# A511-1103/building-detection

Hardware: AMD Instinct MI355X
Metric: 512x512 tiles/sec fwd+bwd DeepLabv3+ (v3plus.py) (full train step: fwd+loss+bwd+Adam) (higher is better)
Workload: dtype f32; 1 GPU; DeepLabv3+ (v3plus.py) 512x512 bs=16/GPU fp32, train step, single GPU; global_batch=16, train_step=one hipGraph replay per step (compile(jit_compile=True)), side_stream_filter_gradients=True

## Files before the change

### building_detection_amd/_lib.py

```python
from __future__ import annotations

import ctypes as C
import os
import threading

_HERE = os.path.dirname(os.path.abspath(__file__))
LIB_PATH = os.path.join(_HERE, "libsegengine.so")

SG_F32, SG_BF16, SG_I64 = 0, 1, 2
SG_HEAD_F32 = 0x100
SG_COMM_ID_BYTES = 128
SG_EPI_BIAS, SG_EPI_RELU = 1, 2
SG_PRO_UP2, SG_EPI_DOWN2 = 16, 32
SG_X_UP2 = 0x200
SG_ACT_RELU, SG_ACT_SIGMOID = 0, 1
SG_LOSS_CE2, SG_LOSS_FOCAL, SG_LOSS_EDGE_FOCAL = 0, 1, 2
SG_MAX_CLASSES = 32
SG_AUGMENT_MAX_ITEMS = 64
SG_AUG_FLIP_UD, SG_AUG_FLIP_LR, SG_AUG_SWAP_RB, SG_AUG_THRESHOLD = 1, 2, 4, 8
SG_SCENE_MAX_ITEMS = 64
SG_SYM_FLIP_UD, SG_SYM_FLIP_LR, SG_SYM_TRANSPOSE = 1, 2, 4
SG_OPT_ADAM, SG_OPT_SGD = 0, 1
SG_OPT_AMSGRAD, SG_OPT_NESTEROV, SG_OPT_EMA = 1, 2, 4
SG_OPT_CLIP_NONE, SG_OPT_CLIP_VALUE, SG_OPT_CLIP_NORM, SG_OPT_CLIP_GLOBAL = 0, 1, 2, 3
# ... 227 lines not shown

_SIGNATURES = {
    "sg_abi_version": (_i, []),
    "sg_last_error": (C.c_char_p, []),
    "sg_set_conv_x6": (_i, [_i]),
    "sg_create": (_i, [_i, _pp]),
    "sg_destroy": (_i, [_vp]),
    "sg_num_cus": (_i, [_vp]),
    "sg_conv2d_fwd": (_i, [_vp, _vp, _i, _dp, _vp, _vp, _vp, _vp, _i, _op]),
    "sg_conv2d_fwd_ws_bytes": (_sz, [_dp]),
    "sg_conv2d_fwd_stats_bytes": (_sz, [_dp]),
    "sg_get_conv_x6": (_i, []),
    "sg_conv2d_planes_job": (_i, [_vp, _i, _dp, _i, C.POINTER(PlanesJob), C.POINTER(C.c_size_t)]),
    "sg_prepare_planes": (_i, [_vp, _vp, _vp, _vp, _vp, _i, _i]),
    "sg_bn_tiles_ws_bytes": (_sz, [_vp, _i, _i]),
    "sg_bn_train_fwd_tiles": (_i, [_vp, _vp, _i, _i64, _i, _vp, _i, _vp, _vp, _vp, _vp, C.c_float, C.c_float, _i, _vp, _sz]),
    "sg_bn_apply": (_i, [_vp, _vp, _i, _i64, _i, _vp, _vp, _vp, _vp, _vp, _vp, _i]),
    "sg_conv2d_dgrad_ws_bytes": (_sz, [_dp]),
    "sg_conv2d_dgrad": (_i, [_vp, _vp, _i, _dp, _vp, _vp, _vp, _vp, _i, _op]),
    "sg_conv2d_wgrad_ws_bytes": (_sz, [_vp, _dp]),
    "sg_conv2d_wgrad": (_i, [_vp, _vp, _i, _dp, _vp, _vp, _vp, _vp, _op]),
    "sg_conv2d_caps": (_i, [_vp, _i, _dp, _i, C.POINTER(ConvCaps)]),
    "sg_conv2d_plan": (_i, [_vp, _i, _dp, _i, _i, _i, C.POINTER(ConvPlan)]),
    "sg_split_planes": (_i, [_vp, _vp, _vp, _i64, _i, _i, _vp]),
    "sg_conv2d_wgrad_planes_ws_bytes": (_sz, [_vp, _dp]),
    "sg_conv2d_wgrad_planes": (_i, [_vp, _vp, _dp, _vp, _vp, _vp, _vp, _sz]),
    "sg_conv2d_wgrad_plan": (_i, [_vp, _i, _dp, _i, _i, C.POINTER(WgradPlan)]),
    "sg_bias_grad_ws_bytes": (_sz, [_vp, _i64, _i]),
    "sg_bias_grad": (_i, [_vp, _vp, _i, _i64, _i, _i, _vp, _vp, _vp, _sz]),
    "sg_dwconv2d_fwd": (_i, [_vp, _vp, _i, _dp, _vp, _vp, _vp, _i, C.POINTER(BnIn)]),
    "sg_dwconv2d_dgrad": (_i, [_vp, _vp, _i, _dp, _vp, _vp, _vp, _vp, _i, _vp, C.POINTER(DwBnSums)]),
    "sg_dwconv2d_dgrad_bnsums_ws_bytes": (_sz, [_vp, _dp]),
    "sg_dwconv2d_wgrad_ws_bytes": (_sz, [_vp, _dp]),
    "sg_dwconv2d_wgrad": (_i, [_vp, _vp, _i, _dp, _vp, _vp, _vp, _i, C.POINTER(BnIn), _vp, _sz]),
    "sg_dwconv2d_plan": (_i, [_vp, _i, _dp, _i, _i, _i, C.POINTER(DwPlan)]),
    "sg_dense_fwd": (_i, [_vp, _vp, _i, _i, _i, _i, _vp, _vp, _vp, _vp, _i]),
    "sg_bn_ws_bytes": (_sz, [_vp, _i64, _i]),
    "sg_bn_train_fwd": (_i, [_vp, _vp, _i, _i64, _i, _vp, _vp, _vp, _vp, _vp, _vp, _vp, _vp, _f, _f, _i, _i, _vp, _sz]),
    "sg_bn_train_bwd": (_i, [_vp, _vp, _i, _i64, _i, _vp, _vp, _vp, _vp, _vp, _vp, _vp, _vp, _vp, _vp, _i, _vp, _sz]),
    "sg_bn_train_bwd_apply": (_i, [_vp, _vp, _i, _i64, _i] + [_vp] * 9 + [_i]),
    "sg_bn_train_bwd_thin_ok": (_i, [_vp, _i, _i64, _i, _i, _i]),
    "sg_bn_train_bwd_thin": (_i, [_vp, _vp, _i, _i64, _i, _i, _i] + [_vp] * 10 + [_i, _vp, _sz]),
    "sg_bn_infer": (_i, [_vp, _vp, _i, _i64, _i, _vp, _vp, _vp, _vp, _vp, _vp, _f, _i]),
    "sg_add2_bn": (_i, [_vp, _vp, _i, _i64, _i] + [_vp] * 11 + [_i, _i, _f, _i, _i]),
    "sg_bn_plan": (_i, [_vp, _i, _i64, _i, _i, _i, C.POINTER(BnPlan)]),
    "sg_seg_plan": (_i, [_vp, _i, _i, _i64, _i, _i, _i, C.POINTER(SegPlan)]),
# ... 146 lines not shown
```

### building_detection_amd/csrc/conv_common.h

```cpp
#pragma once
#include "sg_common.h"
#include <stdlib.h>
#include <string.h>
#include <type_traits>

namespace sgconv {

constexpr int BM = 128;
constexpr int BK = 32;
constexpr int LDA = BK + 4;

template <int V>
using IC = std::integral_constant<int, V>;

struct BnIn {
  const float* mean;
  const float* invstd;
  const float* gamma;
  const float* beta;
  int relu, infer;
  float eps;
};
__device__ __forceinline__ f32x4 bn_in_inv(const BnIn& b, int c) {
  f32x4 is = *reinterpret_cast<const f32x4*>(b.invstd + c);
// ... 27 lines not shown
  const float* __restrict__ bias;
  float* __restrict__ y;
  int H, W, C, x_ld;
  int OH, OW;
  int Nout, y_ld;
  int a_mul, k_mul, off_h, off_w, div;
  int K, M;
  int flags;
  int stagger;
  int ablate;
  uint32_t x_bytes, w_bytes;
  int skip_taps;
  int group_m;
  int cb;
  FastDiv fd_ohow, fd_ow, fd_c, fd_kw;
  const unsigned short* __restrict__ wq;
  int Kpad, Npad;
  int kd;
  float* __restrict__ stats;
  int perm2;
  FastDiv fd_mc, fd_hcwc, fd_wc;
  const float* res;
  const unsigned short* a_planes;
  BnIn bn;
  BnBwdIn bnb;
};

__device__ __forceinline__ int spt_of(const IgemmParams& p) { return p.C / BK; }

__device__ __forceinline__ void row_to_pixel(const IgemmParams& p, uint32_t m, uint32_t& n, uint32_t& oh, uint32_t& ow) {
  if (p.perm2) {
    uint32_t cls, r, rem, i, j;
    fd_divmod(m, p.fd_mc, cls, r);
    fd_divmod(r, p.fd_hcwc, n, rem);
    fd_divmod(rem, p.fd_wc, i, j);
    oh = 2 * i + (cls >> 1);
    ow = 2 * j + (cls & 1);
  } else {
    uint32_t rem;
    fd_divmod(m, p.fd_ohow, n, rem);
    fd_divmod(rem, p.fd_ow, oh, ow);
  }
}
__device__ __forceinline__ int64_t row_to_yoff(const IgemmParams& p, int row) {
  if (!p.perm2) return (int64_t)row * p.y_ld;
  uint32_t n, oh, ow;
  row_to_pixel(p, (uint32_t)row, n, oh, ow);
  return ((int64_t)(n * p.OH + oh) * p.OW + ow) * p.y_ld;
}

struct WgradParams {
  const float* __restrict__ x;
  const float* __restrict__ dy;
  float* __restrict__ out;
  int H, W, Cin, x_ld;
  int OH, OW, Cout, y_ld;
  int stride, dil, pad_t, pad_l;
  int K, P;
  int slabs_per_split;
  int stagger;
  uint32_t x_bytes, dy_bytes;
  int skip_slabs;
  int KH_KW;
  int tap_inner;
  uint32_t x_plane_bytes, dy_plane_bytes;
  BnIn bn;
  int up;
  FastDiv fd_ohow, fd_ow, fd_c, fd_kw, fd_oh;
};

typedef __bf16 bf16x8_t __attribute__((ext_vector_type(8)));
// ... 95 lines not shown
  plan_common(p, vec, bn);
  return bn;
}

enum ConvFamily {
  CONV_NATIVE,
  CONV_THIN,
  CONV_HEAD,
  CONV_SLAB,
  CONV_PATCH,
  CONV_WIDE
};
constexpr int PLAN_NOT_THIN = 1 << 30;

struct ConvPlan {
  ConvFamily family = CONV_NATIVE;
  int nb = 0;
  bool vec = false;
  int perm2 = 0;
  int npl = 0, Ck = 0, Ckp = 0, K = 0, kd = 0, Kpad = 0, Npad = 0, nblocks = 0;
  int wbn = 0;
  size_t w_bytes = 0;
  int x6w_S = 0, b16w_S = 0;
  bool deep = false;
  size_t a_img_bytes = 0, part_img_bytes = 0;
  bool res = false;
  bool bn_in = false;
  bool up2 = false;
  bool bnb = false;
  bool planes_in = false;

  size_t scratch_bytes(int images) const {
    return (((size_t)images * a_img_bytes + 255) & ~(size_t)255) + (size_t)images * part_img_bytes;
  }
  size_t ws_bytes(int images) const {
    const size_t sc = scratch_bytes(images);
    return sc ? ((w_bytes + 255) & ~(size_t)255) + sc : w_bytes;
  }
};

inline SlabKernel slab_kernel_of(const ConvPlan& pl, bool b16, bool with_res) {
  if (pl.npl == 3 && !b16 && pl.x6w_S > 0 && !with_res) return SLAB_X6W;
  if (b16 && pl.deep) return (pl.b16w_S > 0 && !with_res) ? SLAB_B16W : SLAB_B16;
  return SLAB_X6;
}
inline void slab_fill(IgemmParams& p, const ConvPlan& pl) {
// ... 58 lines not shown
```

### building_detection_amd/csrc/conv_igemm.hip

```cpp
#include "conv_common.h"
#include "conv_native.h"
#include "conv_thin.h"
#include "conv_x6p.h"
#include "conv_x6wp.h"

using namespace sgconv;

namespace {

int g_x6_mode = -1;

#include "conv_x6.h"
#include "conv_b16.h"
#include "conv_pw.h"
#include "conv_b16w.h"
#include "conv_x6w.h"

inline int x6_var_of(int64_t tiles, int num_cus) {
  const int var = x6_variant();
  return var < 0 ? ((tiles <= 3 * (int64_t)num_cus) ? 1 : 0) : var;
}
inline bool x6_mf16_of(const IgemmParams& p) { return sg_switch<SW_X6_MF16>() && p.K != p.C; }

template <int NPL, typename TA>
// ... 47 lines not shown
        if constexpr (NPL == 3) {
          if (p.bnb.x)
            return pl.wbn == 256 ? launch_pw_wide<NPL, TA, 256, true>(p, st) : launch_pw_wide<NPL, TA, 384, true>(p, st);
        }
        return pl.wbn == 256 ? launch_pw_wide<NPL, TA, 256>(p, st) : launch_pw_wide<NPL, TA, 384>(p, st);
      }
      break;
    case CONV_SLAB: {
      const int Ck = p.C;
      slab_fill(p, pl);
      p.wq = (const unsigned short*)ws;
      if (!prepared) {
        dim3 grid((unsigned)(p.Kpad / 32), (unsigned)(p.Npad / 32));
        hipLaunchKernelGGL(split3_weights_kernel, grid, dim3(256), 0, st, w, (unsigned short*)ws, pl.K, N, p.Kpad, p.Npad, Ck,
                           Cin * Cout, dgrad ? 1 : Cout, dgrad ? Cout : 1, NPL, pl.Ckp, p.kd);
        SG_LAUNCH_CHECK("split3_weights_kernel");
      }
      char* scratch = (char*)ws + ((pl.w_bytes + 255) & ~(size_t)255);
      const SlabKernel sk = slab_kernel_of(pl, B16, p.res != nullptr);
      if constexpr (NPL == 3 && !B16) {
        if (sk == SLAB_X6W) {
          IgemmParams q = p;
          slab_common(q, sk, 4, num_cus);
          q.ablate = sg_switch<SW_X6W_ABLATE>();
          return launch_x6w(q, pl.x6w_S, scratch, st);
        }
      }
      if constexpr (NPL == 1 && B16) {
        if (sk == SLAB_B16W) {
          IgemmParams q = p;
          slab_common(q, sk, 2, num_cus);
          return launch_b16w(q, pl.b16w_S, pl.b16w_S > 1 ? reinterpret_cast<float*>(scratch) : nullptr, st);
        }
        if (sk == SLAB_B16) return dispatch_b16(p, num_cus, st);
      }
      if (sk != SLAB_X6) break;
      return dispatch_x6<NPL, TA>(p, num_cus, st);
    }
    default:
      break;
  }
  sg_set_error("run_x6: kernel family %d does not read weight planes in this arithmetic (%d planes)", (int)pl.family, NPL);
  return SG_EINVAL;
}

inline size_t x6_ws_bytes(int taps, int C, int N) {
// ... 22 lines not shown
                     int flags, int eb) {
  p.x = (const float*)x;
  p.w = (const float*)w;
  p.bias = (const float*)bias;
  p.y = (float*)y;
  p.H = d->H; p.W = d->W; p.C = d->Cin; p.x_ld = d->x_ld ? d->x_ld : d->Cin;
  p.OH = d->Ho; p.OW = d->Wo;
  p.Nout = d->Cout; p.y_ld = d->y_ld ? d->y_ld : d->Cout;
  p.a_mul = d->stride; p.k_mul = d->dilation; p.off_h = -d->pad_t; p.off_w = -d->pad_l; p.div = 1;
  p.K = d->KH * d->KW * d->Cin;
  p.M = d->N * d->Ho * d->Wo;
  p.flags = flags;
  p.fd_ohow = make_fastdiv((uint32_t)(d->Ho * d->Wo));
  p.fd_ow = make_fastdiv((uint32_t)d->Wo);
  p.fd_c = make_fastdiv((uint32_t)d->Cin);
  p.fd_kw = make_fastdiv((uint32_t)d->KW);
  const int64_t xb = (((int64_t)d->N * d->H * d->W - 1) * p.x_ld + d->Cin) * eb, wb = (int64_t)p.K * d->Cout * 4;
  p.x_bytes = xb < (1ll << 31) ? (uint32_t)xb : 0;
  p.w_bytes = wb < (1ll << 31) ? (uint32_t)wb : 0;
  p.stats = nullptr;
  p.perm2 = 0;
  p.res = nullptr;
  p.a_planes = nullptr;
  p.bn.mean = nullptr;
  p.bnb.x = nullptr;
}

void fill_dgrad_params(IgemmParams& p, const sg_conv_desc* d, const void* dy, const void* wt, const void* bias, void* dx,
                       int flags, int eb) {
  p.x = (const float*)dy;
  p.w = (const float*)wt;
  p.bias = (const float*)bias;
  p.y = (float*)dx;
  p.H = d->Ho; p.W = d->Wo; p.C = d->Cout; p.x_ld = d->y_ld ? d->y_ld : d->Cout;
  p.OH = d->H; p.OW = d->W;
  p.Nout = d->Cin; p.y_ld = d->x_ld ? d->x_ld : d->Cin;
  p.a_mul = 1; p.k_mul = -d->dilation; p.off_h = d->pad_t; p.off_w = d->pad_l; p.div = d->stride;
  p.K = d->KH * d->KW * d->Cout;
  p.M = d->N * d->H * d->W;
  p.flags = flags;
  p.fd_ohow = make_fastdiv((uint32_t)(d->H * d->W));
  p.fd_ow = make_fastdiv((uint32_t)d->W);
  p.fd_c = make_fastdiv((uint32_t)d->Cout);
  p.fd_kw = make_fastdiv((uint32_t)d->KW);
  const int64_t xb = (((int64_t)d->N * d->Ho * d->Wo - 1) * p.x_ld + d->Cout) * eb, wb = (int64_t)p.K * d->Cin * 4;
  p.x_bytes = xb < (1ll << 31) ? (uint32_t)xb : 0;
  p.w_bytes = wb < (1ll << 31) ? (uint32_t)wb : 0;
  p.stats = nullptr;
  p.perm2 = 0;
  p.res = nullptr;
  p.a_planes = nullptr;
  p.bn.mean = nullptr;
  p.bnb.x = nullptr;
}

ConvPlan plan_conv_mode(int mode, int dtype, const sg_conv_desc* d, bool dgrad, int flags) {
  ConvPlan pl;
  const bool b16 = dt_storage(dtype) == SG_BF16, head32 = (dtype & SG_HEAD_F32) != 0;
  const bool f32 = dt_storage(dtype) == SG_F32 && !head32;
  const int eb = dt_bytes(dtype);
  const bool x_dense = !d->x_ld || d->x_ld == d->Cin, y_dense = !d->y_ld || d->y_ld == d->Cout;
  pl.up2 = f32 && mode == 1 && x6p_up2_geom(d) && x6wp_geom(d);
  const bool thin = thin_ok(d) && !(flags & PLAN_NOT_THIN) && !(dgrad && (flags & (SG_EPI_BIAS | SG_EPI_RELU)));
  if (head32) {
    pl.family = thin ? CONV_THIN : CONV_HEAD;
    pl.nb = thin ? d->N : images_per_2gib(d, 2, 4);
    return pl;
  }
  pl.nb = images_per_2gib(d, eb, eb);
  if (thin) {
    pl.family = CONV_THIN;
    pl.res = dgrad;
    pl.bn_in = !dgrad && f32 && !(dtype & SG_X_UP2) && x_dense;
    return pl;
// ... 47 lines not shown
  pl.family = CONV_SLAB;
  pl.res = dgrad;
  pl.deep = b16 && sg_switch<SW_B16_DEEP>();
  pl.kd = x6_plane_kd(b16, pl.Ckp, pl.K == pl.Ckp);
  pl.Kpad = x6_kpad(pl.K, pl.kd);
  pl.Npad = x6_npad(N);
  pl.nblocks = (pl.Kpad / 32) * (pl.Npad / 32);
  pl.w_bytes = x6_planes_bytes(pl.K, N, pl.npl, pl.kd);
  const size_t img_part = (size_t)g.OH * g.OW * N * sizeof(float);
  if (pl.npl == 3 && pl.kd == XW_KD && xw > 0) {
    pl.x6w_S = xw;
    pl.a_img_bytes = (size_t)3 * g.H * g.W * g.C * 2;
    pl.part_img_bytes = xw > 1 ? xw * img_part : 0;
    pl.planes_in = pl.Ckp == pl.Ck && x_dense && y_dense;
  }
  if (pl.deep && pl.kd == BW_KD) {
    pl.b16w_S = b16w_shares(g);
    pl.part_img_bytes = pl.b16w_S > 1 ? pl.b16w_S * img_part : 0;
  }
  return pl;
}

ConvPlan plan_conv(int num_cus, int dtype, const sg_conv_desc* d, bool dgrad, int flags) {
  (void)num_cus;
  return plan_conv_mode(x6_mode(), dtype, d, dgrad, flags);
}

inline void wgrad_extents(int dtype, const sg_conv_desc* d, uint32_t& x_bytes, uint32_t& dy_bytes) {
  const int up = (dtype & SG_X_UP2) ? 1 : 0, eb = dt_bytes(dtype), eby = (dtype & SG_HEAD_F32) ? 4 : eb;
  const int64_t xl = d->x_ld ? d->x_ld : d->Cin, yl = d->y_ld ? d->y_ld : d->Cout;
  const int64_t xb = (((int64_t)d->N * (d->H >> up) * (d->W >> up) - 1) * xl + d->Cin) * eb;
  const int64_t yb = (((int64_t)d->N * d->Ho * d->Wo - 1) * yl + d->Cout) * eby;
  x_bytes = xb < (1ll << 31) ? (uint32_t)xb : 0;
  dy_bytes = yb < (1ll << 31) ? (uint32_t)yb : 0;
}

static int wgrad_slab_split(int num_cus, const sg_conv_desc* d, bool b16) {
  const int64_t K = (int64_t)d->KH * d->KW * d->Cin, P = (int64_t)d->N * d->Ho * d->Wo;
  const int bn = wgrad_bn(d->Cout);
  const int64_t tiles = sg_cdiv(K, BM) * sg_cdiv(d->Cout, bn);
  const int64_t nslab = sg_cdiv(P, BK);
  const int64_t slots = 2 * (int64_t)num_cus;
  const double flops = 2.0 * (double)tiles * BM * bn * (double)P;
  const bool x6_rate = (wgrad_x6_geom(d) || (d->stride == 2 && d->dilation == 1 && d->Wo % BK == 0 && d->Cout >= 16)) && d->Cin % 4 == 0;
  const double rate_x6 = sg_switch_f<SW_WGRAD_PLAN_RATE>() * 1e12;
  const double rate_b16 = sg_switch_f<SW_WGRAD_PLAN_RATE_B16>() * 1e12;
  const double rate = x6_rate ? (b16 ? rate_b16 : rate_x6) : 110e12;
  int64_t maxS = nslab / 8;
// ... 615 lines not shown
  ConvPlan pl = plan_conv(ctx->num_cus, dtype, d, dg, flags);
  if (pl.family == CONV_THIN && !thin_operands_ok(pl, d, aligned == 16, ebx)) pl = plan_conv(ctx->num_cus, dtype, d, dg, flags | PLAN_NOT_THIN);
  if (pl.family == CONV_HEAD) SG_CHECK_ARG(pl.nb >= 1, "%s: one image of the softmax head beyond 2 GiB", who);
  const int nb = (pl.nb >= 1 && pl.nb < d->N) ? pl.nb : d->N;
  const bool fast = pl.family >= CONV_SLAB && pl.vec && aligned == 16;
  sg_conv_plan o;
  memset(&o, 0, sizeof(o));
  o.family = (int)pl.family;
  o.fast = fast;
  o.nb = nb;
  o.nsub = (int)sg_cdiv(d->N, nb);
  o.tail_n = d->N - (o.nsub - 1) * nb;
  o.vec = pl.vec; o.perm2 = pl.perm2; o.npl = pl.npl; o.kd = pl.kd; o.Ck = pl.Ck; o.Ckp = pl.Ckp; o.wbn = pl.wbn;
  o.x6w_S = pl.x6w_S; o.b16w_S = pl.b16w_S; o.deep = pl.deep;
  o.res = pl.res; o.bn_in = pl.bn_in; o.up2 = pl.up2; o.bnb = pl.bnb; o.planes_in = pl.planes_in;
  o.ws_bytes = pl.ws_bytes(nb);
  sg_conv_desc sub = *d;
  sub.N = nb;
  o.main = conv_launch_form(ctx->num_cus, dtype, &sub, pl, fast, dg, aligned, false);
  if (dg && pl.res && !head32 && (pl.family == CONV_THIN || fast)) o.with_res = conv_launch_form(ctx->num_cus, dtype, &sub, pl, fast, dg, aligned, true);
  sub.N = o.tail_n;
  o.tail = conv_launch_form(ctx->num_cus, dtype, &sub, pl, fast, dg, aligned, false);
  *out = o;
  return 0;
}

static int wgrad_plan_checked(const sg_ctx* ctx, int dtype, const sg_conv_desc* d, int ax, int ay, bool planes, const char* who, WgradPlan* pl) {
  SG_CHECK_ARG(ctx != nullptr, "%s: null ctx", who);
  SG_CHECK_ARG(dt_ok(dtype), "%s: dtype %d", who, dtype);
  int rc = check_desc(d, who);
  if (rc) return rc;
  const bool b16 = dt_storage(dtype) == SG_BF16, head32 = (dtype & SG_HEAD_F32) != 0;
  SG_CHECK_ARG(!head32 || (b16 && d->Cout <= 4), "%s: SG_HEAD_F32 needs Cout <= 4 (a softmax head) on bf16 storage", who);
  SG_CHECK_ARG(!planes || (dtype == SG_F32 && ax == 16 && ay == 16), "%s: null / unaligned tensor", who);
  *pl = plan_wgrad(ctx->num_cus, dtype, d, ax, ay, planes);
  if (planes && !pl->main.family) {
    sg_set_error("%s: geometry outside the planes-in kernel (stride 1 SAME, W %% 32 = 0, channels %% 8 = 0, dense "
                 "planes below 2 GiB, not a wide pointwise / patch-form layer, x6 arithmetic)", who);
    return SG_EUNSUPPORTED;
  }
  SG_CHECK_ARG(!(head32 && pl->chunks > 1), "%s: softmax head beyond 2 GiB", who);
  return 0;
}

int sg_conv2d_wgrad_plan(const sg_ctx* ctx, int dtype, const sg_conv_desc* d, int aligned, int planes, sg_wgrad_plan* out) {
  SG_CHECK_ARG(out != nullptr, "sg_conv2d_wgrad_plan: null out");
// ... 214 lines not shown
```

### building_detection_amd/csrc/conv_x6w.h

```cpp
#pragma once

constexpr int XW_M = 128, XW_N = 256, XW_KD = 32, XW_RB = 64;
constexpr int XW_A = 3 * XW_M * XW_RB;
constexpr int XW_B = 3 * XW_N * XW_RB;
constexpr int XW_STAGE = XW_A + XW_B;
constexpr int XW_LDS = 2 * XW_STAGE;

__device__ __forceinline__ int xw_swz(int row) { return (row >> 2) & 3; }

__global__ __launch_bounds__(256) void x6w_split_kernel(const float* __restrict__ x, unsigned short* __restrict__ planes, int64_t rows,
                                                        int C, int x_ld) {
  const int cq = C / 4;
  const int64_t total = rows * cq, plane = rows * (int64_t)C;
  const int64_t stride = (int64_t)gridDim.x * blockDim.x;
  for (int64_t i = (int64_t)blockIdx.x * blockDim.x + threadIdx.x; i < total; i += stride) {
    const int64_t r = i / cq;
    const int c = (int)(i - r * cq) * 4;
    const f32x4 f = *reinterpret_cast<const f32x4*>(x + r * x_ld + c);
    unsigned h0, m0, l0, h1, m1, l1;
    split3_pair(f[0], f[1], h0, m0, l0);
    split3_pair(f[2], f[3], h1, m1, l1);
    unsigned short* dst = planes + r * C + c;
    *reinterpret_cast<u32x2_t*>(dst) = (u32x2_t){h0, h1};
    *reinterpret_cast<u32x2_t*>(dst + plane) = (u32x2_t){m0, m1};
// ... 18 lines not shown
  if (p.group_m > 1) {
    const uint32_t ntm = ntiles / ntn, gm = (uint32_t)p.group_m;
    const uint32_t per = gm * ntn, g = bid / per, r = bid - g * per;
    const uint32_t left = ntm - g * gm, gsz = left < gm ? left : gm;
    tile_n = r / gsz;
    tile_m = g * gm + (r - tile_n * gsz);
  } else {
    tile_m = bid / ntn;
    tile_n = bid - tile_m * ntn;
  }
  const int m0 = tile_m * XW_M, n0 = tile_n * XW_N;

  const __amdgpu_buffer_rsrc_t rsrc_a = __builtin_amdgcn_make_buffer_rsrc(const_cast<unsigned short*>(aq), 0, (int)aq_bytes, 0x00020000);
  const __amdgpu_buffer_rsrc_t rsrc_w =
      __builtin_amdgcn_make_buffer_rsrc(const_cast<unsigned short*>(p.wq), 0, (int)p.w_bytes, 0x00020000);

  const int a_row = wave * 16 + (lane >> 2);
  const int a_chunk = 16 * ((lane & 3) ^ xw_swz(a_row));
  int a_lin = 0, a_hw = (int)0x80008000u;
  {
    const int m = m0 + a_row;
    if (m < p.M) {
      uint32_t n, oh, ow;
      row_to_pixel(p, (uint32_t)m, n, oh, ow);
      const int ohs = (int)oh * p.a_mul + p.off_h, ows = (int)ow * p.a_mul + p.off_w;
      a_lin = (int)n * p.H * p.W + ohs * p.W + ows;
      a_hw = (ohs << 16) | (ows & 0xffff);
    }
  }
  unsigned b_voff[6];
  const int kblocks = p.Kpad >> 5;
#pragma unroll
  for (int j = 0; j < 6; ++j) {
    const int idx = wave + 8 * j;
    const int pl = idx >> 4, rb = idx & 15;
    const int row = rb * 16 + (lane >> 2);
    const int c = (lane & 3) ^ xw_swz(row);
    const int nrow = n0 + row;
    b_voff[j] = nrow < p.Npad ? (unsigned)((((int64_t)pl * kblocks) * p.Npad + nrow) * XW_RB + 16 * c) : OOB;
  }
  auto tap_valid = [&](int dh, int dw, int& pix) -> bool {
    const int ohs = a_hw >> 16, ows = (int)(short)(a_hw & 0xffff);
    const int ih = ohs + dh, iw = ows + dw;
    pix = a_lin + dh * p.W + dw;
    return ((unsigned)ih < (unsigned)p.H) && ((unsigned)iw < (unsigned)p.W);
  };

// ... 174 lines not shown
          __builtin_amdgcn_sched_group_barrier(0x100, 1, 0);
        }
#pragma unroll
        for (int g = 0; g < 9; ++g) {
          __builtin_amdgcn_sched_group_barrier(0x008, 1, 0);
          __builtin_amdgcn_sched_group_barrier(0x020, 1, 0);
        }
        __builtin_amdgcn_sched_group_barrier(0x008, 3, 0);
        __builtin_amdgcn_sched_barrier(0);
      }
      asm volatile("s_waitcnt vmcnt(0)" ::: "memory");
    }
  }

  const bool whole = S == 1;
  const bool has_bias = whole && (p.flags & SG_EPI_BIAS) != 0;
  const bool do_relu = whole && (p.flags & SG_EPI_RELU) != 0;
  {
    float* dst = whole ? p.y : part + (int64_t)split * ((int64_t)p.M * p.Nout);
    const int ld = whole ? p.y_ld : p.Nout;
    const uint32_t obytes = (uint32_t)((((int64_t)p.M - 1) * ld + p.Nout) * 4);
    const __amdgpu_buffer_rsrc_t rsrc_o = __builtin_amdgcn_make_buffer_rsrc(dst, 0, (int)obytes, 0x00020000);
    const unsigned row0 = (unsigned)(m0 + wm + 4 * lh);
#pragma unroll
    for (int j = 0; j < TN; ++j) {
      const int col = n0 + wn + 32 * j + lr;
      const bool cv = col < p.Nout;
      const float bv = has_bias ? p.bias[cv ? col : p.Nout - 1] : 0.f;
      const unsigned cterm = cv ? (unsigned)col * 4u : OOB;
#pragma unroll
      for (int i = 0; i < TM; ++i)
#pragma unroll
        for (int r = 0; r < 16; ++r) {
          const unsigned row = row0 + 32 * i + (r & 3) + 8 * (r >> 2);
          float v = acc[i][j][r] + bv;
          v = do_relu ? fmaxf(v, 0.f) : v;
          unsigned voff = cterm + row * (unsigned)ld * 4u;
          voff = row < (unsigned)p.M ? voff : OOB;
          __builtin_amdgcn_raw_buffer_store_b32(__builtin_bit_cast(unsigned, v), rsrc_o, (int)voff, 0, 0);
        }
    }
  }

  if (whole && p.stats) {
    float* red = reinterpret_cast<float*>(smem);
    float* tmean = red + 2 * XW_N;
    const int nvalid = (p.M - m0) < XW_M ? (p.M - m0) : XW_M;
    const bool hb = (p.flags & SG_EPI_BIAS) != 0;
    __syncthreads();
#pragma unroll
    for (int pass = 0; pass < 2; ++pass) {
#pragma unroll
      for (int j = 0; j < TN; ++j) {
        const int cl = wn + 32 * j + lr;
        const int col = n0 + cl;
        const float bv = (hb && col < p.Nout) ? p.bias[col] : 0.f;
        const float mu = pass ? tmean[cl] : 0.f;
        float sacc = 0.f;
#pragma unroll
        for (int i = 0; i < TM; ++i)
// ... 14 lines not shown
        if (col < p.Nout) p.stats[((int64_t)tile_m * 2 + pass) * p.Nout + col] = tot;
      }
      __syncthreads();
    }
  }
}

inline int x6w_shares(const IgemmParams& p) {
  const int on = sg_switch<SW_X6_WIDE>();
  if (!on) return 0;
  if (p.div != 1 || p.C % XW_KD != 0 || p.K == p.C || p.K < 2048 || p.K / p.C > 64) return 0;
  if (on < 2 && !(p.k_mul > 1 || p.k_mul < -1)) return 0;
  if (p.x_ld % 4 != 0 || p.x_bytes == 0 || p.Nout % 4 != 0) return 0;
  const int64_t ntn = sg_cdiv(p.Nout, XW_N);
  if ((double)p.Nout / (double)(ntn * XW_N) < 0.75) return 0;
  const int64_t img_px = (int64_t)p.OH * p.OW;
  if (img_px < XW_M || img_px % XW_M != 0) return 0;
  const int64_t img_wgs = ntn * (img_px / XW_M);
  if (img_wgs >= 16) return 1;
  if (img_wgs >= 8 && p.K / 2 >= 2048) return 2;
  return 0;
}

inline size_t x6w_a_planes_bytes(const IgemmParams& p) {
  const int64_t batch = p.M / ((int64_t)p.OH * p.OW);
  return (((size_t)3 * (size_t)batch * p.H * p.W * p.C * 2) + 255) & ~(size_t)255;
}

inline int launch_x6w(const IgemmParams& p, int S, char* scratch, hipStream_t st) {
  static bool attr_done = false;
  if (!attr_done) {
    int rc = set_dyn_lds(conv_x6w_kernel<0>, (size_t)XW_LDS);
    if (!rc) rc = set_dyn_lds(conv_x6w_kernel<1>, (size_t)XW_LDS);
    if (rc) return rc;
    attr_done = true;
  }
  const int64_t tiles = sg_cdiv(p.M, XW_M) * sg_cdiv(p.Nout, XW_N);
  const size_t a_bytes = x6w_a_planes_bytes(p);
  const int64_t batch = p.M / ((int64_t)p.OH * p.OW), rows = batch * p.H * p.W;
  const int64_t plane = rows * p.C * 2;
  if (tiles <= 0 || tiles * S > 0x7fffffff || !scratch || 3 * plane >= (1ll << 31) || (((int64_t)p.M - 1) * p.y_ld + p.Nout) * 4 >= (1ll << 31) ||
      (int64_t)p.M * p.Nout * 4 >= (1ll << 31)) {
    sg_set_error("conv_x6w: bad launch (%lld tiles, %d shares) or an operand beyond one 2 GiB buffer descriptor", (long long)tiles, S);
    return SG_EINVAL;
  }
  const unsigned short* aq = p.a_planes;
  if (!aq) {
    int64_t blocks = sg_cdiv(rows * (p.C / 4), 256);
    if (blocks > 16384) blocks = 16384;
    hipLaunchKernelGGL(x6w_split_kernel, dim3((unsigned)blocks), dim3(256), 0, st, p.x, (unsigned short*)scratch, rows, p.C, p.x_ld);
    SG_LAUNCH_CHECK("x6w_split_kernel");
    aq = (const unsigned short*)scratch;
  }
  float* part = S > 1 ? reinterpret_cast<float*>(scratch + a_bytes) : nullptr;
  if (sg_switch<SW_X6W_VAR>() == 1)
    hipLaunchKernelGGL(conv_x6w_kernel<1>, dim3((unsigned)(tiles * S)), dim3(512), (size_t)XW_LDS, st, p, aq,
                       (uint32_t)(3 * plane), (uint32_t)plane, S, part);
  else
    hipLaunchKernelGGL(conv_x6w_kernel<0>, dim3((unsigned)(tiles * S)), dim3(512), (size_t)XW_LDS, st, p, aq,
                       (uint32_t)(3 * plane), (uint32_t)plane, S, part);
  SG_LAUNCH_CHECK("conv_x6w_kernel");
  if (S > 1) {
    dim3 grid((unsigned)sg_cdiv(p.M, 128), (unsigned)sg_cdiv(p.Nout, 64));
    hipLaunchKernelGGL(b16w_reduce_kernel<float>, grid, dim3(256), 0, st, (const float*)part, (p.flags & SG_EPI_BIAS) ? p.bias : nullptr,
                       p.y, p.stats, p.M, p.Nout, p.y_ld, S, (p.flags & SG_EPI_RELU) ? 1 : 0);
    SG_LAUNCH_CHECK("b16w_reduce_kernel<float>");
  }
// ... 3 lines not shown
```

### building_detection_amd/csrc/sg_switch.h

```cpp
#pragma once
#include <stdlib.h>

#define SG_SWITCH_TABLE(X)                                                                                                          \
  X(CONV_X6, INT, 1, "arithmetic of fp32 convolutions: 0 native fp32 MFMA, 1 exact bf16x6 emulation, 2 bf16 products")              \
  X(X6_VARIANT, INT, -1, "x6 structure: 0 two workgroups per CU, 1 one double-buffered workgroup per CU; unset: by tile count")     \
  X(X6_INTERLEAVE, INT, 1, "0: staggered wave halves instead of the hand-interleaved x6 step")                                      \
  X(X6_MF16, OFF0, 1, "0: multi-tap x6 convolutions on the 32x32x16 MFMA instead of 16x16x32")                                      \
  X(X6_VPAD, INT, 1, "0: no virtual channel padding (Cin % 32 != 0 goes to the fp32-MFMA kernels)")                                 \
  X(X6_NOPATCH, FLAG, 0, "patch form of the 3x3 x6 convolution off (im2col x6 kernel instead)")                                     \
  X(X6_NOWPATCH, FLAG, 0, "patch form of the low-channel 3x3 filter gradient off (slab kernel instead)")                            \
  X(X6P_CHUNKS, INT, 1, "0: 3x3 layers of 128 ... 512 channels leave the patch kernel's 64-channel chunks for the im2col kernel")   \
  X(X6P_DELAY, INT, 0, "start offset of a CU's 2nd / 3rd patch workgroup in 10 ns ticks (-1: one K loop)")                          \
  X(X6_WIDE, INT, 2, "planes-in x6 kernel: 2 every long-K multi-tap convolution, 1 the dilated ones only, 0 none")                  \
  X(X6W_VAR, INT, 1, "planes-in x6 kernel: 1 barrier in the middle of a stage, 0 wait + barrier at its end")                        \
  X(CONV_L2, INT, 7, "bit 0 grouped tile order, bit 1 channel-block K order, bit 2 tap-inner wgrad order; unset: 7 on x6, 2 on fp32 kernels") \
  X(CONV_CB, INT, 4, "slabs per channel block of the channel-block K order")                                                        \
  X(CONV_GM, INT, 0, "> 0: row tiles per group of the grouped tile order, for every launch with two or more column tiles")          \
  X(CONV_NOSKIP, FLAG, 0, "padding-tap elimination off")                                                                            \
  X(CONV_NOTHIN, FLAG, 0, "thin 1x1 streaming kernels off")                                                                         \
  X(CONV_MAX_BYTES, INT, 0, "test hook: byte limit above which a convolution call is cut into image sub-batches (<= 0: 2 GiB)")     \
  X(WGRAD_FAST1, FLAG, 0, "aligned-slab form of the fp32 filter gradient off")                                                      \
  X(WGRAD_PLAN_RATE, DBL, 110, "planner's assumed MFMA rate (TFLOP/s) for the x6 filter gradient's split count")                    \
  X(WGRAD_PLAN_RATE_B16, DBL, 110, "planner's assumed MFMA rate (TFLOP/s) for the bf16 filter gradient's split count")              \
  X(WGRAD_PIN_SMUL, INT, 1, "planes-in filter gradient: pixel shares x n")                                                          \
  X(DGRAD_PERM2, INT, 1, "0: stride-2 dgrad rows in raster order instead of parity-class order")                                    \
  X(PW_WIDE, INT, 1, "wide pointwise kernels: 0 off, 2 every aligned 1x1 stride-1 launch (tests), 3 384-wide tiles only")           \
  X(PW_VAR, INT, 1, "pw_wide_kernel<3,float>: 1 barrier in the middle of the k-step, 0 at its end")                                 \
  X(WPW_VAR, INT, 1, "wgrad_pw_wide_kernel: 1 barrier in the middle of the k-step, 0 at its end")                                   \
  X(B16_DEEP, OFF0, 1, "0: bf16 storage on the one-plane x6 kernel instead of conv_b16_kernel")                                     \
  X(B16_KS, INT, 0, "bf16 storage: upper limit of the slab depth in 16-channel units (0: by Cin)")                                  \
  X(B16_PD, INT, 0, "conv_b16_kernel: 1 / 2 register sets of prefetched slabs for every launch (0: by shape)")                      \
  X(B16_WIDE, INT, 1, "0: bf16 storage without the 256-wide LDS-DMA kernel")                                                        \
  X(SEG_FUSED, INT, 1, "segment reductions: 0 separate finalize launch, 1 fused when one workgroup covers a column block, 2 / 3 fused for every split") \
  X(FINALIZE_LANES, INT, 16, "4: four lanes per channel in seg_finalize_kernel whatever the number of partial rows")                \
  X(BN_COLS, INT, 1, "0: flat BatchNormalization apply kernels instead of the column forms")                                        \
  X(DW_STRIP, INT, 1, "0: depthwise filter gradient on the run reducer")                                                            \
  X(DW_RR, INT, 0, "rows per run of the depthwise kernels (1, 2; 0: by shape)")                                                     \
// ... 68 lines not shown
```

### building_detection_amd/switches.py

```python
import os

SWITCHES = {
    "SG_BN_ADD": ("eq1", "1", "BatchNormalization layers in front of a residual Add ride in the add kernel; off: their own launch"),
    "SG_BN_SUMS": ("eq1", "1", "BatchNormalization backward sums come from the depthwise dgrad's epilogue; off: their own reduction"),
    "SG_BN_DEFER": ("eq1", "1", "BatchNormalization(+ReLU) in front of a SeparableConv2D is applied in the depthwise gather"),
    "SG_BN_PW": ("eq1", "0", "the BatchNormalization backward apply rides in the A path of the pointwise dgrad (bit-identical, a loss in the step)"),
    "SG_BN_CONV": ("ne0", "1", "BatchNormalization layers in front of thin 1x1 / patch-kernel convolutions ride in their loader; 0: own launch"),
    "SG_THIN_GRAD_BN": ("ne0", "1", "a thin 1x1 convolution's input gradient is evaluated inside the BatchNormalization backward in front of it; 0: written out"),
    "SG_SCSE_LOWRANK": ("ne0", "1", "an scSE block's input gradient is written once, by a final kernel that adds the two gates' rank-one terms; 0: three passes"),
    "SG_ACT_PLANES": ("ne0", "1", "activation planes made once per tensor and step, kept for the planes-in filter gradient; 0: split in every launch"),
    "SG_UP2_FUSE": ("ne0", "1", "UpSampling2D(2) -> Conv2D 3x3 as one sub-pixel launch; 0: a pair of launches"),
    "SG_GRAD_ACC": ("eq1", "1", "the gradient of a two-consumer block input is summed in the dgrad epilogue; off: by a separate add"),
    "SG_PREPARED_PLANES": ("ne0", "1", "weight planes prepared once per optimiser step; 0: rebuilt inside every convolution call"),
    "SG_JIT_LANES": ("ne0", "1", "the captured training step keeps filter gradients on a side lane; 0: inline in one linear graph"),
    "SG_JIT_LANE_BLOCKS": ("int", "24", "filter-gradient blocks per segment of the captured step's side lane"),
    "SG_SIDE_WGRAD": ("int", "1", "filter gradients on the side stream: 1 all, 2 the GEMM ones only, 3 the depthwise ones only, 0 none"),
    "SG_SIDE_KEEP_GIB": ("float", "4", "GiB of side-stream operands held before the main stream joins the side stream and drops them"),
    "SG_TRACE_MARK": ("eq1", "0", "bracket the roofline kernel set with marker kernels for a kernel trace (read once, at import)"),
    "SG_CONV_NOTHIN": ("flag", "", "thin 1x1 streaming kernels off (the library reads the same variable)"),
    "SG_COMM_INIT_TIMEOUT": ("float", "180", "seconds sg_comm_init may take per rank before every rank gives up together"),
}

_RULES = {
    "eq1": lambda v: v == "1",
    "ne0": lambda v: v != "0",
    "int": int,
    "float": float,
}


def get(name: str):
    kind, default, _ = SWITCHES[name]
    if kind == "flag":
        return name in os.environ
    return _RULES[kind](os.environ.get(name, default))
```

### include/segengine.h

```cpp
#ifndef SEGENGINE_H_
#define SEGENGINE_H_

#include <stddef.h>
#include <stdint.h>

#ifdef __cplusplus
extern "C" {
#endif

#define SG_ABI_VERSION 1

#define SG_EINVAL   (-1)
#define SG_EWORKSPACE (-2)
#define SG_EUNSUPPORTED (-3)
#define SG_ECOMM    (-4)

#define SG_F32  0
#define SG_BF16 1
#define SG_I64  2
#define SG_HEAD_F32 0x100
#define SG_X_UP2 0x200

#define SG_EPI_BIAS 1
#define SG_EPI_RELU 2
// ... 59 lines not shown
#define SG_CF_HEAD 2
#define SG_CF_SLAB 3
#define SG_CF_PATCH 4
#define SG_CF_WIDE 5
#define SG_CK_NATIVE 1
#define SG_CK_THIN 2
#define SG_CK_X6 3
#define SG_CK_B16 4
#define SG_CK_X6W 5
#define SG_CK_B16W 6
#define SG_CK_PATCH 7
#define SG_CK_WIDE 8
typedef struct sg_conv_launch {
  int kernel, bn, vec, ut, var, mf16, ks, pd, skip_taps, group_m, cb, pc, pmulti;
} sg_conv_launch;
typedef struct sg_conv_plan {
  sg_conv_launch main, tail, with_res;
  int family, fast, nb, nsub, tail_n;
  int vec, perm2, npl, kd, Ck, Ckp, wbn, x6w_S, b16w_S, deep;
  int res, bn_in, up2, bnb, planes_in;
  size_t ws_bytes;
} sg_conv_plan;
int sg_conv2d_plan(const sg_ctx* ctx, int dtype, const sg_conv_desc* d, int dgrad, int flags, int aligned, sg_conv_plan* out);

struct sg_bn_in {
  const void* mean;
  const void* invstd;
  const void* gamma;
  const void* beta;
  int32_t relu, infer;
  float eps;
};

struct sg_bn_bwd_in {
  const void* x;
  const void* mean;
  const void* invstd;
  const void* gamma;
  const void* beta;
  const void* dgamma;
  const void* dbeta;
  void* dz;
  int32_t relu;
  int64_t rows;
};

// ... 361 lines not shown
```

Before: 234.3 tiles/s.

## Tile x6w planes-in conv rows as image x row x column blocks to skip dead taps

```diff
diff --git a/building_detection_amd/_lib.py b/building_detection_amd/_lib.py
--- a/building_detection_amd/_lib.py
+++ b/building_detection_amd/_lib.py
@@ -273,6 +273,7 @@
     "sg_conv2d_wgrad": (_i, [_vp, _vp, _i, _dp, _vp, _vp, _vp, _vp, _op]),
     "sg_conv2d_caps": (_i, [_vp, _i, _dp, _i, C.POINTER(ConvCaps)]),
     "sg_conv2d_plan": (_i, [_vp, _i, _dp, _i, _i, _i, C.POINTER(ConvPlan)]),
+    "sg_conv2d_tile_shape": (_i, [_i, _i, _dp, _i, _i, C.POINTER(C.c_int)]),
     "sg_split_planes": (_i, [_vp, _vp, _vp, _i64, _i, _i, _vp]),
     "sg_conv2d_wgrad_planes_ws_bytes": (_sz, [_vp, _dp]),
     "sg_conv2d_wgrad_planes": (_i, [_vp, _vp, _dp, _vp, _vp, _vp, _vp, _sz]),
diff --git a/building_detection_amd/csrc/conv_common.h b/building_detection_amd/csrc/conv_common.h
--- a/building_detection_amd/csrc/conv_common.h
+++ b/building_detection_amd/csrc/conv_common.h
@@ -73,6 +73,8 @@
   FastDiv fd_mc, fd_hcwc, fd_wc;
   const float* res;
   const unsigned short* a_planes;
+  int tile_ni, tile_lth, tile_ltw;
+  FastDiv fd_tct, fd_trt;
   BnIn bn;
   BnBwdIn bnb;
 };
@@ -98,6 +100,16 @@
   uint32_t n, oh, ow;
   row_to_pixel(p, (uint32_t)row, n, oh, ow);
   return ((int64_t)(n * p.OH + oh) * p.OW + ow) * p.y_ld;
+}
+
+__device__ __forceinline__ void row_to_pixel_tiled(const IgemmParams& p, uint32_t m, uint32_t& n, uint32_t& oh, uint32_t& ow) {
+  const uint32_t r = m & 127u, lw = (uint32_t)p.tile_ltw, lh = (uint32_t)p.tile_lth;
+  uint32_t q, ct, g, rt;
+  fd_divmod(m >> 7, p.fd_tct, q, ct);
+  fd_divmod(q, p.fd_trt, g, rt);
+  n = g * (uint32_t)p.tile_ni + (r >> (lw + lh));
+  oh = (rt << lh) + ((r >> lw) & ((1u << lh) - 1u));
+  ow = (ct << lw) + (r & ((1u << lw) - 1u));
 }
 
 struct WgradParams {
@@ -239,6 +251,7 @@
   int wbn = 0;
   size_t w_bytes = 0;
   int x6w_S = 0, b16w_S = 0;
+  int x6w_tile[2][3] = {};
   bool deep = false;
   size_t a_img_bytes = 0, part_img_bytes = 0;
   bool res = false;
diff --git a/building_detection_amd/csrc/conv_igemm.hip b/building_detection_amd/csrc/conv_igemm.hip
--- a/building_detection_amd/csrc/conv_igemm.hip
+++ b/building_detection_amd/csrc/conv_igemm.hip
@@ -93,6 +93,7 @@
         if (sk == SLAB_X6W) {
           IgemmParams q = p;
           slab_common(q, sk, 4, num_cus);
+          x6w_set_tile(q, x6w_tile_of(q, pl.x6w_S, q.stats != nullptr, num_cus));
           q.ablate = sg_switch<SW_X6W_ABLATE>();
           return launch_x6w(q, pl.x6w_S, scratch, st);
         }
@@ -161,6 +162,8 @@
   p.perm2 = 0;
   p.res = nullptr;
   p.a_planes = nullptr;
+  p.tile_ni = p.tile_lth = p.tile_ltw = 0;
+  p.fd_tct = p.fd_trt = make_fastdiv(1);
   p.bn.mean = nullptr;
   p.bnb.x = nullptr;
 }
@@ -189,6 +192,8 @@
   p.perm2 = 0;
   p.res = nullptr;
   p.a_planes = nullptr;
+  p.tile_ni = p.tile_lth = p.tile_ltw = 0;
+  p.fd_tct = p.fd_trt = make_fastdiv(1);
   p.bn.mean = nullptr;
   p.bnb.x = nullptr;
 }
@@ -282,8 +287,21 @@
 }
 
 ConvPlan plan_conv(int num_cus, int dtype, const sg_conv_desc* d, bool dgrad, int flags) {
-  (void)num_cus;
-  return plan_conv_mode(x6_mode(), dtype, d, dgrad, flags);
+  ConvPlan pl = plan_conv_mode(x6_mode(), dtype, d, dgrad, flags);
+  if (pl.family == CONV_SLAB && slab_kernel_of(pl, dt_storage(dtype) == SG_BF16, false) == SLAB_X6W) {
+    sg_conv_desc one = *d;
+    if (pl.nb >= 1 && pl.nb < d->N) one.N = pl.nb;
+    IgemmParams g;
+    if (!dgrad) fill_fwd_params(g, &one, nullptr, nullptr, nullptr, nullptr, 0, dt_bytes(dtype));
+    else fill_dgrad_params(g, &one, nullptr, nullptr, nullptr, nullptr, 0, dt_bytes(dtype));
+    slab_fill(g, pl);
+    slab_common(g, SLAB_X6W, 4, num_cus);
+    for (int st = 0; st < 2; ++st) {
+      const X6wTile t = x6w_tile_of(g, pl.x6w_S, st != 0, num_cus);
+      pl.x6w_tile[st][0] = t.ni; pl.x6w_tile[st][1] = t.th; pl.x6w_tile[st][2] = t.tw;
+    }
+  }
+  return pl;
 }
 
 inline void wgrad_extents(int dtype, const sg_conv_desc* d, uint32_t& x_bytes, uint32_t& dy_bytes) {
@@ -945,6 +963,19 @@
   sub.N = o.tail_n;
   o.tail = conv_launch_form(ctx->num_cus, dtype, &sub, pl, fast, dg, aligned, false);
   *out = o;
+  return 0;
+}
+
+int sg_conv2d_tile_shape(int num_cus, int dtype, const sg_conv_desc* d, int dgrad, int stats, int* out) {
+  SG_CHECK_ARG(out != nullptr, "sg_conv2d_tile_shape: null out");
+  out[0] = out[1] = out[2] = out[3] = 0;
+  SG_CHECK_ARG(num_cus > 0 && dt_ok(dtype) && !(dtype & SG_X_UP2), "sg_conv2d_tile_shape: num_cus %d, dtype %d", num_cus, dtype);
+  int rc = check_desc(d, "sg_conv2d_tile_shape");
+  if (rc) return rc;
+  const ConvPlan pl = plan_conv(num_cus, dtype, d, dgrad != 0, 0);
+  if (pl.family != CONV_SLAB || slab_kernel_of(pl, dt_storage(dtype) == SG_BF16, false) != SLAB_X6W) return 0;
+  const int* t = pl.x6w_tile[stats ? 1 : 0];
+  out[0] = t[0]; out[1] = t[1]; out[2] = t[2]; out[3] = pl.x6w_S;
   return 0;
 }
 
diff --git a/building_detection_amd/csrc/conv_x6w.h b/building_detection_amd/csrc/conv_x6w.h
--- a/building_detection_amd/csrc/conv_x6w.h
+++ b/building_detection_amd/csrc/conv_x6w.h
@@ -64,7 +64,8 @@
     const int m = m0 + a_row;
     if (m < p.M) {
       uint32_t n, oh, ow;
-      row_to_pixel(p, (uint32_t)m, n, oh, ow);
+      if (p.tile_ni) row_to_pixel_tiled(p, (uint32_t)m, n, oh, ow);
+      else row_to_pixel(p, (uint32_t)m, n, oh, ow);
       const int ohs = (int)oh * p.a_mul + p.off_h, ows = (int)ow * p.a_mul + p.off_w;
       a_lin = (int)n * p.H * p.W + ohs * p.W + ows;
       a_hw = (ohs << 16) | (ows & 0xffff);
@@ -285,6 +286,16 @@
     const uint32_t obytes = (uint32_t)((((int64_t)p.M - 1) * ld + p.Nout) * 4);
     const __amdgpu_buffer_rsrc_t rsrc_o = __builtin_amdgcn_make_buffer_rsrc(dst, 0, (int)obytes, 0x00020000);
     const unsigned row0 = (unsigned)(m0 + wm + 4 * lh);
+    unsigned tbase = (unsigned)m0, lw = 7, lhh = 0;
+    if (p.tile_ni) {
+      uint32_t q, ct, g, rt;
+      fd_divmod(tile_m, p.fd_tct, q, ct);
+      fd_divmod(q, p.fd_trt, g, rt);
+      lw = (unsigned)p.tile_ltw;
+      lhh = (unsigned)p.tile_lth;
+      tbase = ((g * (unsigned)p.tile_ni * (unsigned)p.OH + (rt << lhh)) * (unsigned)p.OW) + (ct << lw);
+    }
+    const unsigned mw = (1u << lw) - 1u, mh = (1u << lhh) - 1u, img_rows = (unsigned)(p.OH * p.OW);
 #pragma unroll
     for (int j = 0; j < TN; ++j) {
       const int col = n0 + wn + 32 * j + lr;
@@ -298,7 +309,9 @@
           const unsigned row = row0 + 32 * i + (r & 3) + 8 * (r >> 2);
           float v = acc[i][j][r] + bv;
           v = do_relu ? fmaxf(v, 0.f) : v;
-          unsigned voff = cterm + row * (unsigned)ld * 4u;
+          const unsigned rl = row - (unsigned)m0;
+          const unsigned orow = tbase + (rl >> (lw + lhh)) * img_rows + ((rl >> lw) & mh) * (unsigned)p.OW + (rl & mw);
+          unsigned voff = cterm + orow * (unsigned)ld * 4u;
           voff = row < (unsigned)p.M ? voff : OOB;
           __builtin_amdgcn_raw_buffer_store_b32(__builtin_bit_cast(unsigned, v), rsrc_o, (int)voff, 0, 0);
         }
@@ -359,6 +372,112 @@
   return 0;
 }
 
+struct X6wTile { int ni = 0, th = 0, tw = 0; };
+
+inline int x6w_axis_live(int o0, int on, int a_mul, int off, int k_mul, int nk, int extent) {
+  int live = 0;
+  for (int k = 0; k < nk; ++k) {
+    bool any = false;
+    for (int o = o0; o < o0 + on && !any; ++o) {
+      const int i = o * a_mul + off + k * k_mul;
+      any = i >= 0 && i < extent;
+    }
+    live += any ? 1 : 0;
+  }
+  return live;
+}
+
+inline X6wTile x6w_tile_of(const IgemmParams& p, int S, bool stats, int num_cus) {
+  X6wTile none;
+  if (sg_switch<SW_X6W_TILE>() == 0 || S < 1 || !p.skip_taps || p.perm2 || p.div != 1) return none;
+  if (S == 1 && stats) return none;
+  const int KW = (int)p.fd_kw.d, ntaps = p.K / p.C, KH = ntaps / KW, spt = p.C / XW_KD;
+  const int64_t img_px = (int64_t)p.OH * p.OW;
+  if (KH * KW != ntaps || img_px % XW_M != 0 || p.M % img_px != 0) return none;
+  const int N = (int)(p.M / img_px);
+  if (S > 1) {
+    const int it_run = (p.cb > 0 && spt % p.cb == 0) ? p.cb : spt;
+    if (it_run == spt || spt % (S * it_run) != 0) return none;
+  }
+  const int64_t tiles_m = p.M / XW_M;
+  const bool one_round = tiles_m * sg_cdiv(p.Nout, XW_N) * S <= num_cus;
+  int64_t r_sum = 0;
+  int r_max = 0;
+  for (int64_t m0 = 0; m0 < img_px; m0 += XW_M) {
+    int live = 0;
+    for (int kh = 0; kh < KH; ++kh)
+      for (int kw = 0; kw < KW; ++kw) {
+        bool any = false;
+        for (int r = 0; r < XW_M && !any; ++r) {
+          const int oh = (int)((m0 + r) / p.OW), ow = (int)((m0 + r) % p.OW);
+          const int ih = oh * p.a_mul + p.off_h + kh * p.k_mul, iw = ow * p.a_mul + p.off_w + kw * p.k_mul;
+          any = ih >= 0 && ih < p.H && iw >= 0 && iw < p.W;
+        }
+        live += any ? 1 : 0;
+      }
+    r_sum += live;
+    r_max = live > r_max ? live : r_max;
+  }
+  r_sum *= N;
+  int64_t rs[8], cs[8];
+  int rm[8], cm[8];
+  for (int i = 0; i < 8; ++i) {
+    const int t = 1 << i;
+    rs[i] = cs[i] = -1;
+    rm[i] = cm[i] = 0;
+    if (p.OH % t == 0) {
+      rs[i] = 0;
+      for (int o = 0; o < p.OH; o += t) {
+        const int l = x6w_axis_live(o, t, p.a_mul, p.off_h, p.k_mul, KH, p.H);
+        rs[i] += l;
+        rm[i] = l > rm[i] ? l : rm[i];
+      }
+    }
+    if (p.OW % t == 0) {
+      cs[i] = 0;
+      for (int o = 0; o < p.OW; o += t) {
+        const int l = x6w_axis_live(o, t, p.a_mul, p.off_w, p.k_mul, KW, p.W);
+        cs[i] += l;
+        cm[i] = l > cm[i] ? l : cm[i];
+      }
+    }
+  }
+  X6wTile best;
+  int64_t b_sum = r_sum;
+  int b_max = r_max;
+  for (int li = 0; li < 8; ++li) {
+    const int ni = 1 << li;
+    if (N % ni != 0) continue;
+    for (int lw = 7 - li; lw >= 0; --lw) {
+      const int lh = 7 - li - lw, tw = 1 << lw, th = 1 << lh;
+      if (rs[lh] < 0 || cs[lw] < 0) continue;
+      const int64_t sum = (int64_t)(N / ni) * rs[lh] * cs[lw];
+      const int mx = rm[lh] * cm[lw];
+      const bool better = one_round ? (mx < b_max || (mx == b_max && sum < b_sum)) : sum < b_sum;
+      if (better) {
+        best.ni = ni; best.th = th; best.tw = tw;
+        b_sum = sum;
+        b_max = mx;
+      }
+    }
+  }
+  if (!best.ni) return none;
+  const bool whole_tap = (one_round && b_max < r_max) || r_sum - b_sum >= tiles_m;
+  return whole_tap ? best : none;
+}
+
+inline void x6w_set_tile(IgemmParams& p, const X6wTile& t) {
+  p.tile_ni = 0;
+  p.tile_lth = p.tile_ltw = 0;
+  p.fd_tct = p.fd_trt = make_fastdiv(1);
+  if (!t.ni) return;
+  p.tile_ni = t.ni;
+  while ((1 << p.tile_lth) < t.th) ++p.tile_lth;
+  while ((1 << p.tile_ltw) < t.tw) ++p.tile_ltw;
+  p.fd_tct = make_fastdiv((uint32_t)(p.OW / t.tw));
+  p.fd_trt = make_fastdiv((uint32_t)(p.OH / t.th));
+}
+
 inline size_t x6w_a_planes_bytes(const IgemmParams& p) {
   const int64_t batch = p.M / ((int64_t)p.OH * p.OW);
   return (((size_t)3 * (size_t)batch * p.H * p.W * p.C * 2) + 255) & ~(size_t)255;
@@ -380,6 +499,15 @@
       (int64_t)p.M * p.Nout * 4 >= (1ll << 31)) {
     sg_set_error("conv_x6w: bad launch (%lld tiles, %d shares) or an operand beyond one 2 GiB buffer descriptor", (long long)tiles, S);
     return SG_EINVAL;
+  }
+  if (p.tile_ni) {
+    const int th = 1 << p.tile_lth, tw = 1 << p.tile_ltw;
+    if (p.tile_ni * th * tw != XW_M || batch % p.tile_ni != 0 || p.OH % th != 0 || p.OW % tw != 0 || p.M != batch * p.OH * p.OW ||
+        (S == 1 && p.stats)) {
+      sg_set_error("conv_x6w: tile block %d x %d x %d does not fit %lld images of %d x %d (or statistics in a whole-K launch)", p.tile_ni, th, tw,
+                   (long long)batch, p.OH, p.OW);
+      return SG_EINVAL;
+    }
   }
   const unsigned short* aq = p.a_planes;
   if (!aq) {
diff --git a/building_detection_amd/csrc/sg_switch.h b/building_detection_amd/csrc/sg_switch.h
--- a/building_detection_amd/csrc/sg_switch.h
+++ b/building_detection_amd/csrc/sg_switch.h
@@ -13,6 +13,7 @@
   X(X6P_DELAY, INT, 0, "start offset of a CU's 2nd / 3rd patch workgroup in 10 ns ticks (-1: one K loop)")                          \
   X(X6_WIDE, INT, 2, "planes-in x6 kernel: 2 every long-K multi-tap convolution, 1 the dilated ones only, 0 none")                  \
   X(X6W_VAR, INT, 1, "planes-in x6 kernel: 1 barrier in the middle of a stage, 0 wait + barrier at its end")                        \
+  X(X6W_TILE, INT, 1, "planes-in x6 kernel: 1 tiles as image x row x column blocks where that drops a whole tap, 0 raster rows everywhere") \
   X(CONV_L2, INT, 7, "bit 0 grouped tile order, bit 1 channel-block K order, bit 2 tap-inner wgrad order; unset: 7 on x6, 2 on fp32 kernels") \
   X(CONV_CB, INT, 4, "slabs per channel block of the channel-block K order")                                                        \
   X(CONV_GM, INT, 0, "> 0: row tiles per group of the grouped tile order, for every launch with two or more column tiles")          \
diff --git a/building_detection_amd/switches.py b/building_detection_amd/switches.py
--- a/building_detection_amd/switches.py
+++ b/building_detection_amd/switches.py
@@ -18,6 +18,7 @@
     "SG_SIDE_KEEP_GIB": ("float", "4", "GiB of side-stream operands held before the main stream joins the side stream and drops them"),
     "SG_TRACE_MARK": ("eq1", "0", "bracket the roofline kernel set with marker kernels for a kernel trace (read once, at import)"),
     "SG_CONV_NOTHIN": ("flag", "", "thin 1x1 streaming kernels off (the library reads the same variable)"),
+    "SG_X6W_TILE": ("int", "1", "planes-in x6 kernel: tiles as image x row x column blocks; 0: raster rows (the library reads the same variable)"),
     "SG_COMM_INIT_TIMEOUT": ("float", "180", "seconds sg_comm_init may take per rank before every rank gives up together"),
 }
 
diff --git a/include/segengine.h b/include/segengine.h
--- a/include/segengine.h
+++ b/include/segengine.h
@@ -105,6 +105,8 @@
   size_t ws_bytes;
 } sg_conv_plan;
 int sg_conv2d_plan(const sg_ctx* ctx, int dtype, const sg_conv_desc* d, int dgrad, int flags, int aligned, sg_conv_plan* out);
+
+int sg_conv2d_tile_shape(int num_cus, int dtype, const sg_conv_desc* d, int dgrad, int stats, int* out);
 
 struct sg_bn_in {
   const void* mean;
```

Result: no change. 235.1 tiles/s, median of 6 (+0.3%).
